# hjmkt/wrenc

Hardware: AMD Instinct MI355X
Metric: all-intra encode fps at fixed QP (CTU RD search + final pass); bit-exactness vs the CPU oracle is checked in `parity` (higher is better)
Workload: dtype u8/i16/i32 (+i64 trellis costs, f32 RD cost)

## Files before the change

### wrenc_amd/csrc/dev_common.h

```cpp
#pragma once
#include <cstddef>
#include <type_traits>

#include "dev_const.h"

namespace wrenc {

enum { PLANAR = 0, DC = 1, LT_CCLM = 81, L_CCLM = 82, T_CCLM = 83 };
enum { TREE_SINGLE = 0, TREE_DUAL_LUMA = 1, TREE_DUAL_CHROMA = 2 };

#define GLOBAL_AS __attribute__((address_space(1)))
#define CONST_AS __attribute__((address_space(4)))
#define AS_GLOBAL(T, p) ((GLOBAL_AS T*)(p))
#define LDS_AS __attribute__((address_space(3)))

constexpr int kReconSlots = 4;
constexpr int kSlotBytes = 1536;
__host__ __device__ constexpr int slot_offset(int slot) { return slot < 2 ? slot * kSlotBytes : (slot == 2 ? 2 * kSlotBytes : 2 * kSlotBytes + 384); }
constexpr int kWaveScratch = 2 * kSlotBytes + 384 + 128;

constexpr int kOrgTile = 1536;
constexpr int kBorderBytes = 272;
struct PicBufs {
    const uint8_t* org[3];
// ... 220 lines not shown
        uint32_t lev_was[4];
    };
    union {
        float split_cost[4];
        uint32_t lev_now[4];
    };
    uint8_t ns_luma[4], ns_chroma[4], child[4];
    CtuSt st;
    XRes xr[2];
};

struct Ctx {
    const CONST_AS DevConst* k;
    const GLOBAL_AS uint8_t* org;
    int W, WH;
    uint8_t* pred_scratch;
    GLOBAL_AS uint8_t* slots;
    unsigned long long* mismatch;
    int ctu_x, ctu_y;
    int cu32_mode;
    int write;
    int member;
    int store;
    int solo;
    int trace;
};

#ifndef WRENC_WPB
#define WRENC_WPB 4
#endif
constexpr int WPB = WRENC_WPB;
constexpr int kWorkgroupsPerCU = 20 / WPB;
constexpr int kTeam = 4;
struct LvBox {
    float ns_cost[3], split[3];
    uint8_t ml[3], mc[3];
    uint16_t pad_;
    uint32_t cnt[3][2];
    uint32_t srv_ready, job_posted, job_done, job_ack, job_fin;
    uint32_t job4_posted, job4_done, job4_ack, job4_fin;
    uint8_t job_bx, job_by, job4_bx, job4_by;
};
struct LdsTab {
    int32_t ldq[256];
    int32_t lv[256];
    int8_t fc[32][4];
    LvBox lvb;
#ifdef WRENC_EXP_LDS_PAD
    char pad[WRENC_EXP_LDS_PAD];
#endif
};
__shared__ Lds SHW[WPB];
__shared__ LdsTab SHT;
#define WAVE (__builtin_amdgcn_readfirstlane((int)(threadIdx.x >> 6)))
#define SH (SHW[WAVE])

__device__ __forceinline__ Ctx uni(Ctx c) {
    c.ctu_x = uni(c.ctu_x);
    c.ctu_y = uni(c.ctu_y);
    c.cu32_mode = uni(c.cu32_mode);
    c.write = uni(c.write);
    c.member = uni(c.member);
    c.store = uni(c.store);
    c.solo = uni(c.solo);
    c.trace = uni(c.trace);
    return c;
}

#define WRENC_PRAGMA_(x) _Pragma(#x)
#define WRENC_UNROLL(n) WRENC_PRAGMA_(unroll n)
#ifndef WRENC_U_DCT
#define WRENC_U_DCT 1
#endif
#ifndef WRENC_U_SAD
#define WRENC_U_SAD 0
#endif

#define WSYNC()                                                  \
    do {                                                         \
        __builtin_amdgcn_fence(__ATOMIC_ACQ_REL, "wavefront");   \
        __builtin_amdgcn_wave_barrier();                         \
    } while (0)

#ifdef WRENC_PROFILE
enum { PH_PREDICT, PH_FDCT, PH_QPRE, PH_QBACK, PH_QTRACE, PH_DEQ, PH_IDCT, PH_RECON, PH_TOTAL, PH_CTRL, PH_REFS, PH_SKIP, PH_NSTEP, PH_NFULL, PH_PSZ, PH_PSZ_END = PH_PSZ + 8, PH_PCNT, PH_PCNT_END = PH_PCNT + 8, PH_QB_PRE, PH_QB_WAIT1, PH_QB_WALK, PH_QB_WAIT2, PH_XCHG, PH_COPY, PH_CB, PH_CB_END = PH_CB + 32, PH_CBN, PH_CBN_END = PH_CBN + 32, PH_MEM, PH_MEM_END = PH_MEM + 16, PH_ST, PH_ST_END = PH_ST + 48, PH_STN, PH_STN_END = PH_STN + 12, PH_EV, PH_EV_END = PH_EV + 64, PH_EVN, PH_EVN_END = PH_EVN + 64, PH_QZ, PH_QZ_END = PH_QZ + 4, PH_LEAF, PH_LEAF_END = PH_LEAF + 13, PH_L4, PH_L4_END = PH_L4 + 6, PH_HIST, PH_HIST_END = PH_HIST + 64, PH_CUT, PH_CUT_END = PH_CUT + 8, PH_PRED, PH_PRED_END = PH_PRED + 8, PH_REC, PH_REC_END = PH_REC + 4, PH_SPARSE, PH_SPARSE_END = PH_SPARSE + 16, PH_COUNT };
__device__ unsigned long long g_prof[PH_COUNT];
__shared__ unsigned long long s_prof[PH_COUNT];
#define PROF_T0() const unsigned long long prof_t0_ = __builtin_readcyclecounter()
#define PROF_ADD(ph) do { if (threadIdx.x == 0) s_prof[ph] += __builtin_readcyclecounter() - prof_t0_; } while (0)
#define PROF_MARK(var) const unsigned long long var = __builtin_readcyclecounter()
#define PROF_ADD2(ph, a, b) do { if (threadIdx.x == 0) s_prof[ph] += (b) - (a); } while (0)
#define PROF_CNT(ph, n) do { if (threadIdx.x == 0) s_prof[ph] += (unsigned long long)(n); } while (0)
#define PROF_ADDM(k, a, b) do { if (LANE == 0 && WAVE < 4) s_prof[PH_MEM + 4 * (k) + WAVE] += (b) - (a); } while (0)
#else
#define PROF_ADDM(k, a, b)
#define PROF_T0()
#define PROF_ADD(ph)
#define PROF_MARK(var)
#define PROF_ADD2(ph, a, b)
#define PROF_CNT(ph, n)
#endif

#ifdef WRENC_TRACE
constexpr unsigned kTraceMax = 1u << 19;
__device__ unsigned int g_trace_n;
__device__ int g_trace[kTraceMax * 8];
__device__ __forceinline__ void trace_rec(int x, int y, int lg, int tree, int kind, int ml, int mc, int bits) {
    const unsigned idx = atomicAdd(&g_trace_n, 1u);
    if (idx < kTraceMax) {
        int* r = g_trace + (size_t)idx * 8;
        r[0] = x;
        r[1] = y;
        r[2] = lg;
        r[3] = tree;
        r[4] = kind;
        r[5] = ml;
        r[6] = mc;
        r[7] = bits;
    }
}
#define TRACE_REC(...) trace_rec(__VA_ARGS__)
#else
#define TRACE_REC(...) do { } while (0)
#endif

template <int CTRL>
__device__ __forceinline__ int dpp_mov(int v) {
    return __builtin_amdgcn_mov_dpp(v, CTRL, 0xF, 0xF, true);
}
constexpr int kDppSwap1 = 0xB1;
constexpr int kDppSwap2 = 0x4E;
constexpr int kDppRowHalfMirror = 0x141;
constexpr int kDppRowMirror = 0x140;
__device__ __forceinline__ int row_sum_i32(int v) {
    v += dpp_mov<kDppSwap1>(v);
    v += dpp_mov<kDppSwap2>(v);
    v += dpp_mov<kDppRowHalfMirror>(v);
    v += dpp_mov<kDppRowMirror>(v);
// ... 126 lines not shown
```

### wrenc_amd/csrc/dev_search.h

```cpp
#pragma once

namespace wrenc {

enum { K_SADLIST = 0, K_FULL = 1, K_NOP = 2, K_SADSEARCH = 3, K_CCLMSEARCH = 4, K_SERVE8 = 5, K_LEAF8 = 7, K_LEAF16 = 8, K_SPLIT8 = 9, K_SERVE4 = 10,
       K_NODE8 = 11 };
enum { COPY_NONE = 0, COPY_SAVE = 1, COPY_RESTORE = 2, COPY_PULL = 3 };

#if defined(WRENC_TRACE) || defined(WRENC_EXHAUSTIVE_SPLITS)
constexpr bool kSplitCut = false;
#else
constexpr bool kSplitCut = true;
#endif

#if defined(WRENC_TRACE) || defined(WRENC_EXHAUSTIVE_CANDIDATES)
constexpr bool kCandidateCut = false;
#else
constexpr bool kCandidateCut = true;
#endif

struct Req {
    int kind;
    int comps;
    int tx, ty, tlg;
    int ml, mc;
    bool active;
    bool refs0, refs1;
    bool final;
    int stage;
    int copy_from;
    bool xchg;
    int tree;
    int pre_copy, copy_comps, copy_slot, copy_tx, copy_ty, copy_tlg;
    float fcur;
};

struct Res {
    uint32_t ssd_y, ssd_c;
    long long lvl_y, lvl_c;
    float v0;
    float vmin;
    int imin;
    int imin2;
};
__device__ __forceinline__ Res res_none() {
    Res r;
    r.ssd_y = 0;
    r.ssd_c = 0;
    r.lvl_y = 0;
    r.lvl_c = 0;
    r.v0 = r.vmin = 3.40282347e+38f;
    r.imin = 0;
    r.imin2 = 0;
    return r;
}

__device__ __forceinline__ float uni_f(float v) { return __int_as_float(uni(__float_as_int(v))); }

__device__ __forceinline__ unsigned checksum_weight(int i) { return (2u * (unsigned)i + 1u) * 0x9E3779B1u; }
// ... 209 lines not shown
            const unsigned s4 = (unsigned)__builtin_amdgcn_readlane((int)acc, 4), s5 = (unsigned)__builtin_amdgcn_readlane((int)acc, 5);
            const unsigned c0 = e0 != kNoMode ? s0 : kNoSad, c1 = e1 != kNoMode ? s1 : kNoSad;
            const unsigned mn = min(min(cur, c0), c1);
            int d = 0;
            if (cur == mn) {
            } else if (c0 == mn) {
                d = -2;
                cur = c0;
            } else {
                d = 2;
                cur = c1;
            }
            const int elo = d < 0 ? e2 : (d == 0 ? e3 : e4), ehi = d < 0 ? e3 : (d == 0 ? e4 : e5);
            const unsigned slo = d < 0 ? s2 : (d == 0 ? s3 : s4), shi = d < 0 ? s3 : (d == 0 ? s4 : s5);
            const unsigned p0 = elo != kNoMode ? slo : kNoSad, p1 = ehi != kNoMode ? shi : kNoSad;
            cm += d;
            const unsigned mn2 = min(min(cur, p0), p1);
            if (cur == mn2) {
            } else if (p0 == mn2) {
                cm -= 1;
                cur = p0;
            } else {
                cm += 1;
                cur = p1;
            }
            const int ilo = d < 0 ? 2 : (d == 0 ? 3 : 4);
            traced = traced && (LANE < 2 || LANE == ilo || LANE == ilo + 1);
        } else {
            const unsigned c0 = e0 != kNoMode ? s0 : kNoSad, c1 = e1 != kNoMode ? s1 : kNoSad;
            const unsigned mn = min(min(cur, c0), c1);
            if (cur == mn) {
            } else if (c0 == mn) {
                cm -= st;
                cur = c0;
            } else {
                cm += st;
                cur = c1;
            }
        }
        if (c.trace && traced)
            TRACE_REC(c.ctu_x + q.tx, c.ctu_y + q.ty, q.tlg, q.tree, (q.comps & 1) ? 0 : 2, (q.comps & 1) ? my_mode : 0, my_mode,
                      __float_as_int((float)acc));
    }
    cm_out = cm;
    smin_out = cur;
}

__device__ __forceinline__ Res leaf8_search(const Ctx& c, const Req& q, int* overflow);
__device__ __forceinline__ Res leaf16_search(const Ctx& c, const Req& q, int* overflow);
__device__ __forceinline__ Res split8_search(const Ctx& c, const Req& q, int* overflow, int* leaves = nullptr);
__device__ __forceinline__ void fill_maps(int bx, int by, int lg, int luma_mode, int chroma_mode, bool luma, bool chroma);
__device__ __forceinline__ void serve_pack4(const Ctx& c, const Req& q, int* overflow);
__device__ __forceinline__ void serve_pack8(const Ctx& c, const Req& q, int* overflow);

__device__ __forceinline__ int cclm_probe(const Ctx& c, int tx, int ty, int lg, int tree, CclmParams* all) {
    const int lane = lane_fresh();
    const unsigned acc = sad_list_cclm(c, tx, ty, lg, all);
    const unsigned lt = (unsigned)__builtin_amdgcn_readlane((int)acc, 0), t = (unsigned)__builtin_amdgcn_readlane((int)acc, 1),
                   l = (unsigned)__builtin_amdgcn_readlane((int)acc, 2);
    if (c.trace && lane < 3)
        TRACE_REC(c.ctu_x + tx, c.ctu_y + ty, lg, tree, 2, 0, lane == 0 ? LT_CCLM : (lane == 1 ? T_CCLM : L_CCLM),
                  __float_as_int((float)acc));
    return (lt <= t && lt <= l) ? LT_CCLM : (t <= l ? T_CCLM : L_CCLM);
}

__device__ __forceinline__ int cclm_pred4_lane(const Ctx& c, const Req& q, const CclmPick& pick, int pl, int x, int y) {
    int v = 128;
    if (!pick.flat128) {
        const int ds = cclm_ds6(c, q.tx, q.ty, 2 * y, 2 * x, pick.avail_l);
        v = (M24(ds, pl ? pick.a1 : pick.a0) >> (pl ? pick.k1 : pick.k0)) + (pl ? pick.b1 : pick.b0);
        v = min(max(v, 0), 255);
    }
    return v;
}

__device__ __forceinline__ float node8_search(const Ctx& c, int tx, int ty, int* overflow) {
    Req qn = {};
    qn.comps = 3;
    qn.tx = tx;
    qn.ty = ty;
    qn.tlg = 3;
    qn.refs0 = true;
    qn.refs1 = true;
    qn.tree = TREE_SINGLE;
    stage_org_leaf(c, 3, tx, ty, 3);
    const Res ru = leaf8_search(c, qn, overflow);
    const float ns = ru.vmin;
    const int ml = ru.imin, mc = ru.imin2;
    fill_maps(tx, ty, 3, ml, mc, true, true);
    unsigned kept;
    {
        const int lane = lane_fresh();
        kept = (unsigned)rec_get(0, tx + (lane & 7), ty + (lane >> 3));
        if (lane < 32) kept |= (unsigned)rec_get(1 + (lane >> 4), (tx >> 1) + (lane & 3), (ty >> 1) + ((lane & 15) >> 2)) << 8;
    }
    qn.fcur = ns;
    int leaves = 0;
    const float split8 = split8_search(c, qn, overflow, &leaves).vmin;
    if (!(split8 > ns)) return split8;
    if (leaves) {
        const int lane = lane_fresh();
        rec_put(0, tx + (lane & 7), ty + (lane >> 3), (int)(kept & 255u));
        if (lane < 32) rec_put(1 + (lane >> 4), (tx >> 1) + (lane & 3), (ty >> 1) + ((lane & 15) >> 2), (int)(kept >> 8));
        fill_maps(tx, ty, 3, ml, mc, true, true);
    }
    return ns;
}

template <bool TEAM, bool D3>
__device__ __forceinline__ Res evaluate(const Ctx& c, const PicBufs& pb, const Req& q, int* overflow) {
    Res r = res_none();
    PROF_MARK(tcp0_);
    if (q.pre_copy != COPY_NONE)
        copy_block(c, q.pre_copy, q.copy_comps, q.copy_slot, q.copy_tx, q.copy_ty, q.copy_tlg, q.copy_from);
    PROF_MARK(tcp1_);
    PROF_ADD2(PH_COPY, tcp0_, tcp1_);
    if (q.kind == K_NOP) return r;
    if (q.stage) stage_org_leaf(c, q.stage, q.tx, q.ty, q.tlg);
    constexpr bool kNodes = !TEAM && D3;
    if (kNodes && q.kind == K_NODE8) {
        r.vmin = node8_search(c, q.tx, q.ty, overflow);
        return r;
    }
    if (!kNodes && q.kind == K_LEAF8) return leaf8_search(c, q, overflow);
    if (q.kind == K_LEAF16) return leaf16_search(c, q, overflow);
    if (TEAM && D3 && q.kind == K_SPLIT8) return split8_search(c, q, overflow);
    if (TEAM && q.kind == K_SERVE8) {
        serve_pack8(c, q, overflow);
        return r;
    }
    if (TEAM && D3 && q.kind == K_SERVE4) {
        serve_pack4(c, q, overflow);
        return r;
    }
    int mc = q.mc;
    CclmPick cpick_ = CclmPick{};
    if (q.kind == K_CCLMSEARCH) {
        if (q.tlg > 4) stage_org(c, 2, q.tx, q.ty, q.tlg);
        CclmParams call_;
        mc = cclm_probe(c, q.tx, q.ty, q.tlg, q.tree, &call_);
        r.imin = mc;
        cpick_ = cclm_pick(call_, 2 * cclm_mode_index(mc));
    }
    if (q.kind == K_FULL || q.kind == K_CCLMSEARCH) {
#pragma unroll 1
        for (int round = 0; round < 2; ++round) {
            const int cset = q.comps & (1 << round);
            if (!cset) continue;
            if (q.active) {
#pragma unroll 1
                for (int comp = 0; comp < 2; ++comp)
                    if ((cset >> comp) & 1) {
                        PROF_MARK(tf0_);
                        full_front(c, q, comp, comp ? mc : q.ml, 0, cpick_);
                        PROF_MARK(tf1_);
                        PROF_ADD2(PH_PSZ + ((q.tlg - 2) * 2 + comp), tf0_, tf1_);
                        PROF_ADD2(PH_PCNT + ((q.tlg - 2) * 2 + comp), 0, 1);
                    }
            }
            PROF_MARK(ts0_);
            bool any_y = false, any_c = false;
            {
                bool any = false;
                long long lvl = 0;
                if (q.active)
                    lvl = quantize_solo(c, q.tlg - round, round ? 2 : 1, overflow, &any);
                if (round) {
                    r.lvl_c = lvl;
                    any_c = any;
                } else {
                    r.lvl_y = lvl;
                    any_y = any;
                }
            }
            PROF_MARK(ts1_);
            PROF_ADD2(PH_QZ + ((q.tlg - 2) & 3), ts0_, ts1_);
            if (!q.active) {
                PROF_ADD2(PH_SKIP, ts0_, ts1_);
                continue;
            }
#pragma unroll 1
            for (int comp = 0; comp < 2; ++comp) {
                if (!((cset >> comp) & 1)) continue;
                PROF_MARK(tb0_);
                const uint32_t ssd = full_back(c, pb, q, comp, 0, comp ? any_c : any_y);
                PROF_MARK(tb1_);
                PROF_ADD2(PH_PSZ + ((q.tlg - 2) * 2 + comp), tb0_, tb1_);
                if (comp)
                    r.ssd_c = ssd;
                else
                    r.ssd_y = ssd;
            }
        }
        return r;
    }
    PROF_MARK(tr0_);
    if (q.refs0 && (q.comps & 1)) build_refs(c, 0, q.tx, q.ty, q.tlg);
    if (q.refs1 && (q.comps & 2)) build_refs(c, 1, q.tx, q.ty, q.tlg);
    if (q.tlg > 4) stage_org(c, q.comps, q.tx, q.ty, q.tlg);
    PROF_MARK(t0_);
    PROF_ADD2(PH_REFS, tr0_, t0_);
    if (q.kind == K_SADSEARCH) {
        constexpr unsigned kNoSad = 0xFFFFFFFFu;
        int cm;
        unsigned smin = kNoSad;
        sad_search(c, q, cm, smin);
        r.imin = uni(cm);
        r.vmin = smin == kNoSad ? 3.40282347e+38f : uni_f((float)smin);
    } else {
        PROF_MARK(tp0_);
        const unsigned sad = (unsigned)wave_sum_i32(predict_sad(c, 1, q.tx, q.ty, q.tlg, q.mc));
        PROF_MARK(tp1_);
        PROF_ADD2(PH_PSZ + ((q.tlg - 2) * 2 + 1), tp0_, tp1_);
        PROF_ADD2(PH_PCNT + ((q.tlg - 2) * 2 + 1), 0, 1);
        if (c.trace && LANE == 0)
            TRACE_REC(c.ctu_x + q.tx, c.ctu_y + q.ty, q.tlg, q.tree, 2, 0, q.mc, __float_as_int((float)sad));
        r.v0 = uni_f((float)sad);
    }
    PROF_MARK(t1_);
    PROF_ADD2(PH_PREDICT, t0_, t1_);
    PROF_ADD2(PH_PRED + 7, t0_, t1_);
    return r;
}

__device__ __forceinline__ int nb_luma_mode(Ctx c, int x, int y, bool* exists) {
    if (x >= 0 && y >= 0) {
        *exists = true;
        return c.cu32_mode;
    }
    if (y >= 0 && x < 0 && c.ctu_x > 0) {
        *exists = true;
        return uni((int)SH.left_mode[y >> 2]);
    }
    *exists = false;
    return PLANAR;
}

struct MpmList {
    int k0, k1, k2, k3, k4;
};
__device__ __forceinline__ MpmList mpm_list(const Ctx& c, int bx, int by, int lg) {
    const int n = 1 << lg;
    bool le, ae;
    int left = nb_luma_mode(c, bx - 1, by + n - 1, &le);
    if (!le) left = PLANAR;
    int above;
    if (by - 1 < 0) {
        above = PLANAR;
// ... 727 lines not shown
}

__device__ __forceinline__ Res leaf16_search(const Ctx& c, const Req& q, int* overflow) {
    Res r = res_none();
    const int lane = lane_fresh();
    if (q.refs0) build_refs(c, 0, q.tx, q.ty, 4);
    if (q.refs1) build_refs(c, 1, q.tx, q.ty, 4);
    LeafBest best = leaf_best_init(PLANAR);
    const MpmList mpl_ = mpm_list(c, q.tx, q.ty, 4);
    {
        PROF_MARK(la0_);
        const Pack16Out a = pack16_eval(c, q, 2, PLANAR, DC, overflow);
        leaf_candidate(c, q.tx, q.ty, 4, TREE_SINGLE, mpl_, best, 0, PLANAR, pack_parts(a, 0));
        leaf_candidate(c, q.tx, q.ty, 4, TREE_SINGLE, mpl_, best, 1, DC, pack_parts(a, 1));
        pack16_to_tile(c, q, 2, best.win);
        PROF_MARK(la1_);
        PROF_ADD2(PH_LEAF + 4, la0_, la1_);
    }
    int cm;
    unsigned smin;
    PROF_MARK(ls0_);
    sad_search(c, q, cm, smin);
    PROF_MARK(ls1_);
    PROF_ADD2(PH_LEAF + 5, ls0_, ls1_);
    cm = uni(cm);
    const int lo = !(cm < 3) ? cm - 1 : kNoMode, hi = !(cm + 1 > 66) ? cm + 1 : kNoMode;
    {
        const Pack16Out b = pack16_eval(c, q, 2, cm, lo, overflow);
        best.win = -1;
        leaf_candidate(c, q.tx, q.ty, 4, TREE_SINGLE, mpl_, best, 0, cm, pack_parts(b, 0));
        if (lo != kNoMode) leaf_candidate(c, q.tx, q.ty, 4, TREE_SINGLE, mpl_, best, 1, lo, pack_parts(b, 1));
        if (best.win >= 0) pack16_to_tile(c, q, 2, best.win);
    }
    PROF_MARK(lb1_);
    PROF_ADD2(PH_LEAF + 6, ls1_, lb1_);
    if (hi != kNoMode) {
        const Pack16Out b = pack16_eval(c, q, 1, hi, kNoMode, overflow);
        best.win = -1;
        leaf_candidate(c, q.tx, q.ty, 4, TREE_SINGLE, mpl_, best, 0, hi, pack_parts(b, 0));
        if (best.win >= 0) pack16_to_tile(c, q, 1, best.win);
    }
    PROF_MARK(lc1_);
    PROF_ADD2(PH_LEAF + 7, lb1_, lc1_);
    r.vmin = best.cost;
    r.imin = best.mode;
    r.imin2 = best.mode;
    r.ssd_y = best.e.ssd_y;
    r.ssd_c = best.e.ssd_c;
    r.lvl_y = best.e.lvl_y;
    r.lvl_c = best.e.lvl_c;
    return r;
}

__device__ __forceinline__ void fill_maps(int bx, int by, int lg, int luma_mode, int chroma_mode, bool luma,
                                          bool chroma) {
    const int l4 = lg - 2;
    if (luma && LANE < (1 << (2 * l4))) {
        const int idx = ((by >> 2) + (LANE >> l4)) * 8 + (bx >> 2) + (LANE & ((1 << l4) - 1));
        SH.cu_log2[idx] = (uint8_t)lg;
        SH.luma_mode[idx] = (uint8_t)luma_mode;
    }
    if (chroma) {
        const int l8 = max(l4 - 1, 0);
        if (LANE < (1 << (2 * l8)))
            SH.chroma_mode[((by >> 3) + (LANE >> l8)) * 4 + (bx >> 3) + (LANE & ((1 << l8) - 1))] = (uint8_t)chroma_mode;
    }
    WSYNC();
}


__device__ __forceinline__ bool split_floor_cut(const Ctx& c, float partial, int n, int fi, bool chroma, float unsplit,
                                                float* bound) {
    if (!kSplitCut) return false;
    float b = partial;
    const float f = c.k->split_floor[fi];
    for (int i = 0; i < n; ++i) b = b + f;
    if (chroma) b = b + c.k->split_floor[1];
    b = uni_f(b);
    if (!(b > unsplit)) return false;
    *bound = b;
    return true;
}

__device__ __forceinline__ Res split8_search(const Ctx& c, const Req& q, int* overflow, int* leaves) {
    Res r = res_none();
    float split8 = 0.0f;
#pragma unroll 1
    for (int i8 = 0; i8 < 4; ++i8) {
        Req ql = {};
        ql.comps = 1;
        ql.tx = q.tx + (i8 & 1) * 4;
        ql.ty = q.ty + (i8 >> 1) * 4;
        ql.tlg = 2;
        ql.refs0 = true;
        ql.refs1 = false;
        ql.tree = TREE_DUAL_LUMA;
        if (split_floor_cut(c, split8, 4 - i8, 0, true, q.fcur, &r.vmin)) {
            PROF_ADD2(PH_CUT + 0, 0, 4 - i8);
            PROF_ADD2(PH_CUT + 1, 0, 1);
            PROF_ADD2(PH_CUT + 4, 0, split8 > q.fcur ? 0 : 1);
            return r;
        }
        if (leaves) *leaves = 1;
        PROF_MARK(l4g0_);
        stage_org_leaf(c, 1, ql.tx, ql.ty, 2);
        PROF_MARK(l4g1_);
// ... 6 lines not shown
        PROF_ADD2(PH_CUT + 1, 0, 1);
        PROF_ADD2(PH_CUT + 4, 0, split8 > q.fcur ? 0 : 1);
        return r;
    }
    Req qc = {};
    qc.tx = q.tx;
    qc.ty = q.ty;
    qc.comps = 2;
    qc.tlg = 3;
    qc.ml = 0;
    qc.mc = uni((int)SH.luma_mode[((q.ty + 4) >> 2) * 8 + ((q.tx + 4) >> 2)]);
    qc.refs0 = false;
    qc.refs1 = true;
    qc.tree = TREE_DUAL_CHROMA;
    PROF_MARK(l4c0_);
    stage_org_leaf(c, 2, q.tx, q.ty, 3);
    const Res rc = leafc4_search(c, qc, overflow);
    fill_maps(q.tx, q.ty, 3, 0, rc.imin, false, true);
    PROF_MARK(l4c1_);
    PROF_ADD2(PH_L4 + 4, l4c0_, l4c1_);
    r.vmin = uni_f(split8 + rc.vmin);
    return r;
}

__device__ __forceinline__ void req_full(Req& q, int comps, int tx, int ty, int tlg, int ml, int mc, bool active,
                                         bool refs0, bool refs1, bool final) {
    q.kind = K_FULL;
    q.comps = comps;
    q.tx = tx;
    q.ty = ty;
    q.tlg = tlg;
    q.ml = ml;
    q.mc = mc;
    q.active = active;
    q.refs0 = refs0;
    q.refs1 = refs1;
    q.final = final;
    q.stage = (final && tlg <= 4) ? comps : 0;
    q.pre_copy = COPY_NONE;
    q.xchg = false;
}

__device__ __forceinline__ void req_copy(Req& q, int mode, int comps, int slot, int tx, int ty, int tlg) {
    q.pre_copy = mode;
    q.copy_comps = comps;
    q.copy_slot = slot;
    q.copy_tx = tx;
    q.copy_ty = ty;
    q.copy_tlg = tlg;
    q.copy_from = -1;
}

enum {
    C_START = 0, C_PLANAR = 1, C_DCM = 2, C_LIST = 3, C_F0 = 6, C_F1 = 7, C_F2 = 8, C_CCLM = 11, C_DM = 12,
    C_L8 = 20, C_L16 = 21, C_WINNER = 22
};

__device__ __forceinline__ void leaf_init(LeafSt& s, int bx, int by, int lg, int slot = 0) {
    s.cont = C_START;
    s.bx = (uint8_t)bx;
    s.by = (uint8_t)by;
    s.lg = (uint8_t)lg;
    s.need_refs0 = 1;
    s.need_refs1 = 1;
    s.need_org = lg <= 4 ? 1 : 0;
    s.need_save = 0;
    s.tile_best = 0;
    s.slot = (uint8_t)slot;
}

__device__ __forceinline__ void leaf_attach_save(LeafSF& s, Req& q) {
    q.pre_copy = COPY_NONE;
    if (s.need_save) {
        req_copy(q, COPY_SAVE, 3, s.slot, s.bx, s.by, s.lg);
        s.need_save = 0;
    }
}
__device__ __forceinline__ void leaf_attach_org(LeafSF& s, Req& q) {
    q.stage = 0;
    if (s.need_org) {
        q.stage = 3;
        s.need_org = 0;
    }
}
__device__ __forceinline__ void leaf_copy_only(LeafSF& s, Req& q, int mode, int comps, int cont) {
    q.kind = K_NOP;
    q.xchg = false;
    req_copy(q, mode, comps, s.slot, s.bx, s.by, s.lg);
    s.cont = (uint8_t)cont;
}

__device__ __forceinline__ void leaf_full(LeafSF& s, Req& q, int comps, int ml, int mc, bool act, int cont) {
    const bool r0 = (comps & 1) && s.need_refs0 != 0;
    const bool r1 = (comps & 2) && mc < LT_CCLM && s.need_refs1 != 0;
    req_full(q, comps, s.bx, s.by, s.lg, ml, mc, act, r0, r1, false);
    q.tree = TREE_SINGLE;
    leaf_attach_org(s, q);
    leaf_attach_save(s, q);
    if (act) {
        if (r0) s.need_refs0 = 0;
        if (r1) s.need_refs1 = 0;
    }
    s.op_ml = (uint8_t)ml;
    s.op_mc = (uint8_t)mc;
    s.op_act = act ? 1 : 0;
    s.cont = (uint8_t)cont;
}
// ... 23 lines not shown
    q.kind = K_SADSEARCH;
    q.xchg = false;
    q.tree = TREE_SINGLE;
    q.comps = 3;
    q.tx = s.bx;
    q.ty = s.by;
    q.tlg = s.lg;
    q.refs0 = s.need_refs0 != 0;
    q.refs1 = s.need_refs1 != 0;
    if (q.refs0) s.need_refs0 = 0;
    if (q.refs1) s.need_refs1 = 0;
    leaf_attach_org(s, q);
    leaf_attach_save(s, q);
    s.cont = (uint8_t)cont;
}

__device__ __forceinline__ void leaf_leaf8(LeafSF& s, Req& q, int cont) {
    req_full(q, 3, s.bx, s.by, s.lg, 0, 0, true, s.need_refs0 != 0, s.need_refs1 != 0, false);
    q.kind = K_LEAF8;
    q.tree = TREE_SINGLE;
    leaf_attach_org(s, q);
    leaf_attach_save(s, q);
    s.need_refs0 = 0;
    s.need_refs1 = 0;
    s.cont = (uint8_t)cont;
}

__device__ __forceinline__ void leaf_leaf16(LeafSF& s, Req& q, int cont) {
    leaf_leaf8(s, q, cont);
    q.kind = K_LEAF16;
}

__device__ __forceinline__ EvalParts res_parts(const Res& r) {
    EvalParts e;
    e.ssd_y = r.ssd_y;
    e.ssd_c = r.ssd_c;
    e.lvl_y = r.lvl_y;
    e.lvl_c = r.lvl_c;
    return e;
}
__device__ __forceinline__ void put_parts(EvalPartsSF& d, const EvalParts& e) {
    d.ssd_y = e.ssd_y;
    d.ssd_c = e.ssd_c;
    d.lvl_y = e.lvl_y;
    d.lvl_c = e.lvl_c;
}

__device__ __forceinline__ void leaf_take(LeafSF& s, float val, const EvalParts& parts, int mode, int cls) {
    s.best_cost = val;
    put_parts(s.e_best, parts);
    s.mode = (uint8_t)mode;
    s.best_cls = (uint8_t)cls;
}
__device__ __forceinline__ void leaf_offer(LeafSF& s, float val, const EvalParts& parts, int mode, int cls) {
    if (val < s.best_cost) {
        leaf_take(s, val, parts, mode, cls);
        s.need_save = 1;
        s.tile_best = 1;
    } else if (s.op_act) {
        s.tile_best = 0;
    }
}

__device__ __forceinline__ bool leaf_step(const Ctx& c, LeafSF& s, const Res& r, Req& q) {
    constexpr int tree = TREE_SINGLE;
    int cont = s.cont;
    float val = 0.0f;
    int cls = 0;
    const EvalParts rp = res_parts(r);
    if (cont == C_PLANAR || cont == C_DCM || cont == C_F0 || cont == C_F1 || cont == C_F2) {
        if (s.op_act) {
            cls = mpm_class(c, s.bx, s.by, s.lg, s.op_ml);
            val = uni_f(assemble_cost(c, tree, cls, s.op_mc, rp));
            if (c.trace && LANE == 0)
                TRACE_REC(c.ctu_x + s.bx, c.ctu_y + s.by, s.lg, tree, 1, s.op_ml, s.op_mc, __float_as_int(val));
        } else {
            val = 3.40282347e+38f;
        }
    }
    for (;;) {
        switch (cont) {
        case C_START:
            if (s.lg == 3) {
                leaf_leaf8(s, q, C_L8);
                return true;
            }
            if (s.lg == 4) {
                leaf_leaf16(s, q, C_L16);
                return true;
            }
            leaf_full(s, q, 3, PLANAR, PLANAR, true, C_PLANAR);
            return true;
        case C_L16:
            leaf_take(s, r.vmin, rp, r.imin, mpm_class(c, s.bx, s.by, s.lg, r.imin));
            s.need_save = 1;
            s.tile_best = 1;
            cont = C_WINNER;
            break;
        case C_L8:
            s.cost = r.vmin;
            s.luma_mode = (uint8_t)r.imin;
            s.chroma_mode = (uint8_t)r.imin2;
            return false;
        case C_PLANAR:
            leaf_take(s, val, rp, PLANAR, cls);
            s.need_save = 1;
            s.tile_best = 1;
            leaf_full(s, q, 3, DC, DC, true, C_DCM);
            return true;
        case C_DCM:
            leaf_offer(s, val, rp, DC, cls);
            leaf_sadsearch(s, q, C_LIST);
            return true;
        case C_LIST: {
            const int cm = r.imin;
            s.cur_mode = (uint8_t)cm;
            s.cur_cost = r.vmin;
            leaf_full(s, q, 3, cm, cm, true, C_F0);
            return true;
        }
        case C_F0: {
            const int cm = s.cur_mode;
            leaf_offer(s, val, rp, cm, cls);
            leaf_full(s, q, 3, cm - 1, cm - 1, !(cm < 3), C_F1);
            return true;
        }
        case C_F1: {
            const int cm = s.cur_mode;
            leaf_offer(s, val, rp, cm - 1, cls);
            leaf_full(s, q, 3, cm + 1, cm + 1, !(cm + 1 > 66), C_F2);
            return true;
        }
        case C_F2:
            leaf_offer(s, val, rp, s.cur_mode + 1, cls);
            cont = C_WINNER;
            break;
        case C_WINNER: {
            s.cost = s.best_cost;
            const int m = s.mode;
            s.luma_mode = (uint8_t)m;
            s.chroma_mode = (uint8_t)m;
            const bool in_tile = s.tile_best != 0;
            s.cur_cost = uni_f(assemble_chroma_cost(c, m, s.e_best.get()));
            if (c.trace && LANE == 0)
                TRACE_REC(c.ctu_x + s.bx, c.ctu_y + s.by, s.lg, tree, 3, 0, m, __float_as_int((float)s.cur_cost));
            leaf_cclmsearch(s, q, C_CCLM);
            if (!in_tile) req_copy(q, COPY_RESTORE, 1, s.slot, s.bx, s.by, s.lg);
            return true;
        }
        case C_CCLM: {
            s.cclm_mode = (uint8_t)r.imin;
            EvalParts e = s.e_best.get();
            e.ssd_c = rp.ssd_c;
            e.lvl_c = rp.lvl_c;
            const float cclm_cost = uni_f(assemble_chroma_cost(c, s.cclm_mode, e));
            if (c.trace && LANE == 0)
                TRACE_REC(c.ctu_x + s.bx, c.ctu_y + s.by, s.lg, tree, 3, 0, s.cclm_mode, __float_as_int(cclm_cost));
            const int m = s.mode;
            const int bcls = s.best_cls;
            if (dm_keeps(s.cur_cost, cclm_cost)) {
                s.cost = uni_f(assemble_cost(c, tree, bcls, m, s.e_best.get()));
                leaf_copy_only(s, q, COPY_RESTORE, 2, C_DM);
                return true;
            }
            s.chroma_mode = s.cclm_mode;
            s.cost = uni_f(assemble_cost(c, tree, bcls, s.cclm_mode, e));
            return false;
        }
        default:
            return false;
        }
    }
}



__device__ __forceinline__ EvalParts xparts(const Ctx& c, int par, int m) {
    const XRes& x = team_lds(c, m).xr[par];
    EvalParts e;
    e.ssd_y = (uint32_t)uni((int)x.ssd_y);
    e.ssd_c = (uint32_t)uni((int)x.ssd_c);
    e.lvl_y = uni_i64(x.lvl_y);
    e.lvl_c = uni_i64(x.lvl_c);
    return e;
}
__device__ __forceinline__ float xvmin(const Ctx& c, int par, int m) { return __int_as_float(uni((int)team_lds(c, m).xr[par].ssd_y)); }
__device__ __forceinline__ int ximin(const Ctx& c, int par, int m) { return uni((int)team_lds(c, m).xr[par].ssd_c); }
__device__ __forceinline__ float xv0(const Ctx& c, int par, int m) { return __int_as_float(uni((int)team_lds(c, m).xr[par].lvl_y)); }

// ... 213 lines not shown
    const int lg = tlg - 1;
    const int cwords = 1 << (2 * lg - 2);
    for (int w = LANE; w < 2 * cwords; w += 64) {
        const int pl = w >= cwords ? 1 : 0;
        const int ww = w - pl * cwords;
        const int row = (4 * ww) >> lg, col = (4 * ww) & ((1 << lg) - 1);
        const int at = ((ty >> 1) + row) * 20 + (tx >> 1) + col + 4;
        *(uint32_t*)&SH.recC[pl][at] = *(const uint32_t*)&src.recC[pl][at];
    }
    WSYNC();
}
__device__ __forceinline__ float lv_decide(const Ctx& c, int L, int idx) {
    const int me = c.member;
    const int dl = c.k->max_depth;
    const int nmem = L == 0 ? kTeam : dl - L + 1;
    PROF_MARK(tx0_);
    lv_meet(L, 0, (idx + 1) * nmem);
    PROF_MARK(tx1_);
    PROF_ADD2(PH_XCHG, tx0_, tx1_);
    PROF_ADDM(2, tx0_, tx1_);
    const float ns = uni_f(SHT.lvb.ns_cost[L]), sp = uni_f(SHT.lvb.split[L]);
    const int ml = uni((int)SHT.lvb.ml[L]), mc = uni((int)SHT.lvb.mc[L]);
    int bx, by;
    lv_node(L, idx, bx, by);
    const int lg = 5 - L;
    const bool unsplit = sp > ns;
    if (unsplit) {
        if (me > L) lv_pull(c, L, bx, by, lg);
        fill_maps(bx, by, lg, ml, mc, true, true);
    } else if (me == L || me > dl) {
        lv_pull(c, L + 1, bx, by, lg);
        lv_pull_maps(c, L + 1, bx, by, lg);
    }
    PROF_MARK(tx2_);
    lv_meet(L, 1, (idx + 1) * nmem);
    PROF_MARK(tx3_);
    PROF_ADD2(PH_COPY, tx1_, tx2_);
    PROF_ADD2(PH_XCHG, tx2_, tx3_);
    PROF_ADDM(2, tx2_, tx3_);
    return unsplit ? ns : sp;
}
__device__ __forceinline__ void lv_post_unsplit(int L, float ns, int ml, int mc) {
    if (LANE == 0) {
        SHT.lvb.ns_cost[L] = ns;
        SHT.lvb.ml[L] = (uint8_t)ml;
        SHT.lvb.mc[L] = (uint8_t)mc;
    }
}
__device__ __forceinline__ void lv_post_split(int L, float sp) {
    if (LANE == 0) SHT.lvb.split[L] = sp;
}


enum { T_START = 0, T_ENTER = 1, T_NODE_LEAF = 2, T_NODE8 = 3, T_REGEN_DONE = 6, T_RETURN = 7, T_FINAL_Z = 8, T_FZ_TAIL = 9, T_FZ_NEXT = 10,
       T_LV_UNIT = 11, T_LV_LEAFDONE = 12, T_LV_UP = 13, T_SPLIT8 = 14, T_LV_SERVE = 15 };

template <bool TEAM, bool D3>
__device__ __forceinline__ bool ctu_step(Ctx& c, const Res& r, Req& q) {
    CtuSt& t = SH.st;
    bool in_leaf = t.in_leaf != 0;
    int cont = t.cont;
    for (;;) {
        if (in_leaf) {
            LeafSF ls = snap_leaf(t.leaf);
            if ((TEAM && !t.lvmode) ? leaf_step_team(c, t, ls, q, t.xpar ^ 1, r) : leaf_step(c, ls, r, q)) {
                if (t.pend) {
                    req_copy(q, COPY_SAVE, t.pend, t.pslot, t.pbx, t.pby, t.plg);
                    t.pend = 0;
                }
                t.cont = (uint8_t)cont;
                t.in_leaf = 1;
                return true;
            }
            t.in_leaf = 0;
            in_leaf = false;
        }
        switch (cont) {
        case T_START:
            t.level = 0;
            t.bx = 0;
            t.by = 0;
            cont = T_ENTER;
            break;
        case T_ENTER: {
            const int lg = 5 - t.level;
            t.lg = (uint8_t)lg;
            if (!TEAM && D3 && lg == 3) {
                req_full(q, 3, t.bx, t.by, 3, 0, 0, true, false, false, false);
                q.kind = K_NODE8;
                q.tree = TREE_SINGLE;
                if (t.pend) {
                    req_copy(q, COPY_SAVE, t.pend, t.pslot, t.pbx, t.pby, t.plg);
                    t.pend = 0;
                }
                t.cont = T_NODE8;
                return true;
            }
            leaf_init(t.leaf, t.bx, t.by, lg, (!TEAM && t.level < t.max_depth) ? 1 + t.level : 0);
            if (TEAM && !t.lvmode) t.leaf.cont = TC_START;
            in_leaf = true;
            cont = T_NODE_LEAF;
            break;
        }
        case T_NODE_LEAF: {
            const float ns = t.leaf.cost;
            const int ml = t.leaf.luma_mode, mc = t.leaf.chroma_mode;
            const int level = t.level, lg = t.lg;
            fill_maps(t.bx, t.by, lg, ml, mc, true, true);
            if (level == 0) c.cu32_mode = ml;
            if (t.max_depth - level == 0) {
                t.ret = ns;
                cont = T_RETURN;
                break;
            }
            if (TEAM) {
                if (t.dp0) {
                    const int dp = t.dp0, dq = t.dp1;
                    t.dp0 = 0;
                    copy_block(c, COPY_PULL, (dp >> 1) & 3, 0, (dq & 7) << 2, (dq >> 3) << 2, (dp >> 5) + 2, (dp >> 3) & 3);
                }
                t.lvmode = 1;
                t.lv_i = 0;
                t.lv_acc0 = 0.0f;
                t.lv_acc1 = 0.0f;
                if (c.member == 0) lv_post_unsplit(0, ns, ml, mc);
                cont = (c.member == 0 || c.member > t.max_depth) ? T_LV_UP : T_LV_UNIT;
                break;
            }
            t.pend = (uint8_t)(mc >= LT_CCLM ? 2 : 0);
            t.pbx = t.bx;
            t.pby = t.by;
            t.plg = (uint8_t)lg;
            t.pslot = (uint8_t)(1 + level);
            if (LANE == 0) {
                SH.ns_cost[level] = ns;
                SH.ns_luma[level] = (uint8_t)ml;
                SH.ns_chroma[level] = (uint8_t)mc;
                SH.split_cost[level] = 0.0f;
                SH.child[level] = 0;
            }
            WSYNC();
            float bound;
            if (split_floor_cut(c, 0.0f, 4, 2 + level + 1, false, ns, &bound)) {
                PROF_ADD2(PH_CUT + 2 + level, 0, 4);
                PROF_ADD2(PH_CUT + 5, 0, 1);
                t.pend = 0;
                t.ret = ns;
                cont = T_RETURN;
                break;
            }
            t.level = (uint8_t)(level + 1);
            cont = T_ENTER;
            break;
        }
        case T_NODE8: {
            if constexpr (!TEAM && D3) {
                t.ret = r.vmin;
                cont = T_RETURN;
                break;
            }
            }
            break;
        case T_SPLIT8: {
            if constexpr (TEAM && D3) {
                lv_post_split(2, r.vmin);
                cont = T_LV_UP;
                break;
            }
            }
            break;
        case T_REGEN_DONE:
            fill_maps(t.rbx, t.rby, t.rlg, t.rl, t.rc, true, true);
            t.ret = uni_f(SH.ns_cost[t.level]);
            cont = T_RETURN;
            break;
        case T_RETURN: {
            const int level = t.level;
            if (level == 0) {
                t.ctu_cost = t.ret;
                t.z = 0;
                if (TEAM && t.dp0) {
                    q.kind = K_NOP;
                    q.pre_copy = COPY_NONE;
                    q.xchg = false;
                    t.cont = T_RETURN;
                    return true;
                }
                t.z = (uint8_t)(TEAM ? 16 * c.member : 0);
                t.zend = (uint8_t)(TEAM ? 16 * c.member + 16 : 64);
                cont = T_FINAL_Z;
                break;
            }
            const int pl = level - 1;
            const int psz = 1 << (5 - pl);
            const int pbx = t.bx & ~(psz - 1), pby = t.by & ~(psz - 1);
            const float acc = uni_f(uni_f(SH.split_cost[pl]) + t.ret);
            const int ch = uni((int)SH.child[pl]) + 1;
            WSYNC();
            if (LANE == 0) {
                SH.split_cost[pl] = acc;
                SH.child[pl] = (uint8_t)ch;
            }
            WSYNC();
            const float ns_p = uni_f(SH.ns_cost[pl]);
            float bound;
            const bool lost = ch < 4 ? split_floor_cut(c, acc, 4 - ch, 2 + level, false, ns_p, &bound) : acc > ns_p;
            if (ch < 4 && !lost) {
// ... 385 lines not shown
```

Baseline: 277.0.

## Run the 32x32 leaf search as one fused device request instead of state-machine steps

Adds a K_LEAF32 request kind that evaluates the whole 32x32 leaf (planar, DC, SAD search, the cm±1 neighbours, then DM vs CCLM chroma) inside a single full_search call. Previously each candidate was a separate request that returned through the ctu_step/leaf_step state machine. The aim is to cut per-request dispatch, state save/restore and snapshot overhead at the CTU level. It removes the old C_PLANAR..C_F2 leaf states and adds profiling slots plus an LDS size static_assert, at the cost of more code and register pressure in the solo path.

```diff
diff --git a/wrenc_amd/csrc/dev_common.h b/wrenc_amd/csrc/dev_common.h
--- a/wrenc_amd/csrc/dev_common.h
+++ b/wrenc_amd/csrc/dev_common.h
@@ -296,6 +296,9 @@
 };
 __shared__ Lds SHW[WPB];
 __shared__ LdsTab SHT;
+#if !defined(WRENC_EXP_LDS_PAD) && WRENC_WPB == 4
+static_assert(sizeof(Lds) * WPB + sizeof(LdsTab) == 31968, "the workgroup's LDS is 31,968 bytes");
+#endif
 #define WAVE (__builtin_amdgcn_readfirstlane((int)(threadIdx.x >> 6)))
 #define SH (SHW[WAVE])
 
@@ -327,7 +330,7 @@
     } while (0)
 
 #ifdef WRENC_PROFILE
-enum { PH_PREDICT, PH_FDCT, PH_QPRE, PH_QBACK, PH_QTRACE, PH_DEQ, PH_IDCT, PH_RECON, PH_TOTAL, PH_CTRL, PH_REFS, PH_SKIP, PH_NSTEP, PH_NFULL, PH_PSZ, PH_PSZ_END = PH_PSZ + 8, PH_PCNT, PH_PCNT_END = PH_PCNT + 8, PH_QB_PRE, PH_QB_WAIT1, PH_QB_WALK, PH_QB_WAIT2, PH_XCHG, PH_COPY, PH_CB, PH_CB_END = PH_CB + 32, PH_CBN, PH_CBN_END = PH_CBN + 32, PH_MEM, PH_MEM_END = PH_MEM + 16, PH_ST, PH_ST_END = PH_ST + 48, PH_STN, PH_STN_END = PH_STN + 12, PH_EV, PH_EV_END = PH_EV + 64, PH_EVN, PH_EVN_END = PH_EVN + 64, PH_QZ, PH_QZ_END = PH_QZ + 4, PH_LEAF, PH_LEAF_END = PH_LEAF + 13, PH_L4, PH_L4_END = PH_L4 + 6, PH_HIST, PH_HIST_END = PH_HIST + 64, PH_CUT, PH_CUT_END = PH_CUT + 8, PH_PRED, PH_PRED_END = PH_PRED + 8, PH_REC, PH_REC_END = PH_REC + 4, PH_SPARSE, PH_SPARSE_END = PH_SPARSE + 16, PH_COUNT };
+enum { PH_PREDICT, PH_FDCT, PH_QPRE, PH_QBACK, PH_QTRACE, PH_DEQ, PH_IDCT, PH_RECON, PH_TOTAL, PH_CTRL, PH_REFS, PH_SKIP, PH_NSTEP, PH_NFULL, PH_PSZ, PH_PSZ_END = PH_PSZ + 8, PH_PCNT, PH_PCNT_END = PH_PCNT + 8, PH_QB_PRE, PH_QB_WAIT1, PH_QB_WALK, PH_QB_WAIT2, PH_XCHG, PH_COPY, PH_CB, PH_CB_END = PH_CB + 32, PH_CBN, PH_CBN_END = PH_CBN + 32, PH_MEM, PH_MEM_END = PH_MEM + 16, PH_ST, PH_ST_END = PH_ST + 48, PH_STN, PH_STN_END = PH_STN + 12, PH_EV, PH_EV_END = PH_EV + 64, PH_EVN, PH_EVN_END = PH_EVN + 64, PH_QZ, PH_QZ_END = PH_QZ + 4, PH_LEAF, PH_LEAF_END = PH_LEAF + 16, PH_L4, PH_L4_END = PH_L4 + 6, PH_HIST, PH_HIST_END = PH_HIST + 64, PH_CUT, PH_CUT_END = PH_CUT + 8, PH_PRED, PH_PRED_END = PH_PRED + 8, PH_REC, PH_REC_END = PH_REC + 4, PH_SPARSE, PH_SPARSE_END = PH_SPARSE + 16, PH_COUNT };
 __device__ unsigned long long g_prof[PH_COUNT];
 __shared__ unsigned long long s_prof[PH_COUNT];
 #define PROF_T0() const unsigned long long prof_t0_ = __builtin_readcyclecounter()
diff --git a/wrenc_amd/csrc/dev_search.h b/wrenc_amd/csrc/dev_search.h
--- a/wrenc_amd/csrc/dev_search.h
+++ b/wrenc_amd/csrc/dev_search.h
@@ -3,7 +3,7 @@
 namespace wrenc {
 
 enum { K_SADLIST = 0, K_FULL = 1, K_NOP = 2, K_SADSEARCH = 3, K_CCLMSEARCH = 4, K_SERVE8 = 5, K_LEAF8 = 7, K_LEAF16 = 8, K_SPLIT8 = 9, K_SERVE4 = 10,
-       K_NODE8 = 11 };
+       K_NODE8 = 11, K_LEAF32 = 12 };
 enum { COPY_NONE = 0, COPY_SAVE = 1, COPY_RESTORE = 2, COPY_PULL = 3 };
 
 #if defined(WRENC_TRACE) || defined(WRENC_EXHAUSTIVE_SPLITS)
@@ -319,6 +319,8 @@
 __device__ __forceinline__ void fill_maps(int bx, int by, int lg, int luma_mode, int chroma_mode, bool luma, bool chroma);
 __device__ __forceinline__ void serve_pack4(const Ctx& c, const Req& q, int* overflow);
 __device__ __forceinline__ void serve_pack8(const Ctx& c, const Req& q, int* overflow);
+template <bool TEAM, bool L32>
+__device__ __forceinline__ Res full_search(const Ctx& c, const PicBufs& pb, const Req& q, int* overflow);
 
 __device__ __forceinline__ int cclm_probe(const Ctx& c, int tx, int ty, int lg, int tree, CclmParams* all) {
     const int lane = lane_fresh();
@@ -400,67 +402,9 @@
         serve_pack4(c, q, overflow);
         return r;
     }
-    int mc = q.mc;
-    CclmPick cpick_ = CclmPick{};
-    if (q.kind == K_CCLMSEARCH) {
-        if (q.tlg > 4) stage_org(c, 2, q.tx, q.ty, q.tlg);
-        CclmParams call_;
-        mc = cclm_probe(c, q.tx, q.ty, q.tlg, q.tree, &call_);
-        r.imin = mc;
-        cpick_ = cclm_pick(call_, 2 * cclm_mode_index(mc));
-    }
-    if (q.kind == K_FULL || q.kind == K_CCLMSEARCH) {
-#pragma unroll 1
-        for (int round = 0; round < 2; ++round) {
-            const int cset = q.comps & (1 << round);
-            if (!cset) continue;
-            if (q.active) {
-#pragma unroll 1
-                for (int comp = 0; comp < 2; ++comp)
-                    if ((cset >> comp) & 1) {
-                        PROF_MARK(tf0_);
-                        full_front(c, q, comp, comp ? mc : q.ml, 0, cpick_);
-                        PROF_MARK(tf1_);
-                        PROF_ADD2(PH_PSZ + ((q.tlg - 2) * 2 + comp), tf0_, tf1_);
-                        PROF_ADD2(PH_PCNT + ((q.tlg - 2) * 2 + comp), 0, 1);
-                    }
-            }
-            PROF_MARK(ts0_);
-            bool any_y = false, any_c = false;
-            {
-                bool any = false;
-                long long lvl = 0;
-                if (q.active)
-                    lvl = quantize_solo(c, q.tlg - round, round ? 2 : 1, overflow, &any);
-                if (round) {
-                    r.lvl_c = lvl;
-                    any_c = any;
-                } else {
-                    r.lvl_y = lvl;
-                    any_y = any;
-                }
-            }
-            PROF_MARK(ts1_);
-            PROF_ADD2(PH_QZ + ((q.tlg - 2) & 3), ts0_, ts1_);
-            if (!q.active) {
-                PROF_ADD2(PH_SKIP, ts0_, ts1_);
-                continue;
-            }
-#pragma unroll 1
-            for (int comp = 0; comp < 2; ++comp) {
-                if (!((cset >> comp) & 1)) continue;
-                PROF_MARK(tb0_);
-                const uint32_t ssd = full_back(c, pb, q, comp, 0, comp ? any_c : any_y);
-                PROF_MARK(tb1_);
-                PROF_ADD2(PH_PSZ + ((q.tlg - 2) * 2 + comp), tb0_, tb1_);
-                if (comp)
-                    r.ssd_c = ssd;
-                else
-                    r.ssd_y = ssd;
-            }
-        }
-        return r;
-    }
+    if (!TEAM && q.kind == K_LEAF32) return full_search<TEAM, true>(c, pb, q, overflow);
+    if (q.kind == K_FULL || q.kind == K_CCLMSEARCH) return full_search<TEAM, false>(c, pb, q, overflow);
+    if constexpr (!TEAM) return r;
     PROF_MARK(tr0_);
     if (q.refs0 && (q.comps & 1)) build_refs(c, 0, q.tx, q.ty, q.tlg);
     if (q.refs1 && (q.comps & 2)) build_refs(c, 1, q.tx, q.ty, q.tlg);
@@ -1294,6 +1238,151 @@
     return r;
 }
 
+template <bool TEAM, bool L32>
+__device__ __forceinline__ Res full_search(const Ctx& c, const PicBufs& pb, const Req& q, int* overflow) {
+    Res r = res_none();
+    constexpr bool l32 = !TEAM && L32;
+    const int tx = l32 ? 0 : q.tx, ty = l32 ? 0 : q.ty, tlg = l32 ? 5 : q.tlg;
+    Req qe = {};
+    qe.tx = tx;
+    qe.ty = ty;
+    qe.tlg = tlg;
+    qe.tree = q.tree;
+    qe.final = q.final;
+    qe.comps = q.comps;
+    qe.ml = q.ml;
+    qe.active = q.active;
+    qe.refs0 = q.refs0;
+    qe.refs1 = q.refs1;
+    int mc = q.mc;
+    CclmPick cpick_ = CclmPick{};
+    LeafBest best = leaf_best_init(PLANAR);
+    MpmList mpl_ = {};
+    int cm = 0;
+    bool tile_best = false;
+    float dm_cost = 0.0f;
+    if (l32) mpl_ = mpm_list(c, tx, ty, tlg);
+    constexpr int steps = l32 ? 6 : 1;
+#pragma unroll 1
+    for (int k = 0; k < steps; ++k) {
+        PROF_MARK(lk0_);
+        bool probe = !l32 && q.kind == K_CCLMSEARCH;
+        if (l32 && (k == 3 ? cm < 3 : (k == 4 && cm + 1 > 66))) continue;
+        if (l32) {
+            if (k == 2) {
+                PROF_MARK(ls0_);
+                stage_org(c, 3, tx, ty, tlg);
+                unsigned smin;
+                sad_search(c, qe, cm, smin);
+                cm = uni(cm);
+                PROF_MARK(ls1_);
+                PROF_ADD2(PH_LEAF + 14, ls0_, ls1_);
+            }
+            const int mode = k == 0 ? PLANAR : (k == 1 ? DC : (k == 2 ? cm : (k == 3 ? cm - 1 : cm + 1)));
+            qe.ml = mode;
+            mc = mode;
+            qe.refs0 = qe.refs1 = k == 0;
+            if (k == 5) {
+                if (!tile_best) copy_block(c, COPY_RESTORE, 1, q.copy_slot, tx, ty, tlg);
+                dm_cost = uni_f(assemble_chroma_cost(c, best.mode, best.e));
+                if (c.trace && LANE == 0)
+                    TRACE_REC(c.ctu_x + tx, c.ctu_y + ty, tlg, TREE_SINGLE, 3, 0, best.mode, __float_as_int(dm_cost));
+                qe.comps = 2;
+                qe.ml = 0;
+                probe = true;
+            }
+        }
+        PROF_MARK(lkc_);
+        if (probe) {
+            if (tlg > 4) stage_org(c, 2, tx, ty, tlg);
+            CclmParams call_;
+            mc = cclm_probe(c, tx, ty, tlg, q.tree, &call_);
+            r.imin = mc;
+            cpick_ = cclm_pick(call_, 2 * cclm_mode_index(mc));
+        }
+#pragma unroll 1
+        for (int round = 0; round < 2; ++round) {
+            const int cset = qe.comps & (1 << round);
+            if (!cset) continue;
+            if (qe.active) {
+#pragma unroll 1
+                for (int comp = 0; comp < 2; ++comp)
+                    if ((cset >> comp) & 1) {
+                        PROF_MARK(tf0_);
+                        full_front(c, qe, comp, comp ? mc : qe.ml, 0, cpick_);
+                        PROF_MARK(tf1_);
+                        PROF_ADD2(PH_PSZ + ((tlg - 2) * 2 + comp), tf0_, tf1_);
+                        PROF_ADD2(PH_PCNT + ((tlg - 2) * 2 + comp), 0, 1);
+                    }
+            }
+            PROF_MARK(ts0_);
+            bool any_y = false, any_c = false;
+            {
+                bool any = false;
+                long long lvl = 0;
+                if (qe.active)
+                    lvl = quantize_solo(c, tlg - round, round ? 2 : 1, overflow, &any);
+                if (round) {
+                    r.lvl_c = lvl;
+                    any_c = any;
+                } else {
+                    r.lvl_y = lvl;
+                    any_y = any;
+                }
+            }
+            PROF_MARK(ts1_);
+            PROF_ADD2(PH_QZ + ((tlg - 2) & 3), ts0_, ts1_);
+            if (!qe.active) {
+                PROF_ADD2(PH_SKIP, ts0_, ts1_);
+                continue;
+            }
+#pragma unroll 1
+            for (int comp = 0; comp < 2; ++comp) {
+                if (!((cset >> comp) & 1)) continue;
+                PROF_MARK(tb0_);
+                const uint32_t ssd = full_back(c, pb, qe, comp, 0, comp ? any_c : any_y);
+                PROF_MARK(tb1_);
+                PROF_ADD2(PH_PSZ + ((tlg - 2) * 2 + comp), tb0_, tb1_);
+                if (comp)
+                    r.ssd_c = ssd;
+                else
+                    r.ssd_y = ssd;
+            }
+        }
+        if (!l32) continue;
+        EvalParts e;
+        e.ssd_y = r.ssd_y;
+        e.ssd_c = r.ssd_c;
+        e.lvl_y = r.lvl_y;
+        e.lvl_c = r.lvl_c;
+        if (k < 5) {
+            tile_best = leaf_candidate(c, tx, ty, tlg, TREE_SINGLE, mpl_, best, k, qe.ml, e);
+            if (tile_best) copy_block(c, COPY_SAVE, 3, q.copy_slot, tx, ty, tlg);
+            PROF_MARK(lk1_);
+            PROF_ADD2(PH_LEAF + 13, lkc_, lk1_);
+            continue;
+        }
+        const int cclm = mc;
+        e.ssd_y = best.e.ssd_y;
+        e.lvl_y = best.e.lvl_y;
+        const float cclm_cost = uni_f(assemble_chroma_cost(c, cclm, e));
+        if (c.trace && LANE == 0)
+            TRACE_REC(c.ctu_x + tx, c.ctu_y + ty, tlg, TREE_SINGLE, 3, 0, cclm, __float_as_int(cclm_cost));
+        r.imin = best.mode;
+        if (dm_keeps(dm_cost, cclm_cost)) {
+            r.vmin = uni_f(assemble_cost(c, TREE_SINGLE, best.cls, best.mode, best.e));
+            r.imin2 = best.mode;
+            copy_block(c, COPY_RESTORE, 2, q.copy_slot, tx, ty, tlg);
+        } else {
+            r.vmin = uni_f(assemble_cost(c, TREE_SINGLE, best.cls, cclm, e));
+            r.imin2 = cclm;
+        }
+        PROF_MARK(lk2_);
+        PROF_ADD2(PH_LEAF + 15, lk0_, lk2_);
+    }
+    return r;
+}
+
 __device__ __forceinline__ void fill_maps(int bx, int by, int lg, int luma_mode, int chroma_mode, bool luma,
                                           bool chroma) {
     const int l4 = lg - 2;
@@ -1406,7 +1495,7 @@
 }
 
 enum {
-    C_START = 0, C_PLANAR = 1, C_DCM = 2, C_LIST = 3, C_F0 = 6, C_F1 = 7, C_F2 = 8, C_CCLM = 11, C_DM = 12,
+    C_START = 0, C_CCLM = 11, C_DM = 12,
     C_L8 = 20, C_L16 = 21, C_WINNER = 22
 };
 
@@ -1536,32 +1625,10 @@
     s.mode = (uint8_t)mode;
     s.best_cls = (uint8_t)cls;
 }
-__device__ __forceinline__ void leaf_offer(LeafSF& s, float val, const EvalParts& parts, int mode, int cls) {
-    if (val < s.best_cost) {
-        leaf_take(s, val, parts, mode, cls);
-        s.need_save = 1;
-        s.tile_best = 1;
-    } else if (s.op_act) {
-        s.tile_best = 0;
-    }
-}
-
 __device__ __forceinline__ bool leaf_step(const Ctx& c, LeafSF& s, const Res& r, Req& q) {
     constexpr int tree = TREE_SINGLE;
     int cont = s.cont;
-    float val = 0.0f;
-    int cls = 0;
     const EvalParts rp = res_parts(r);
-    if (cont == C_PLANAR || cont == C_DCM || cont == C_F0 || cont == C_F1 || cont == C_F2) {
-        if (s.op_act) {
-            cls = mpm_class(c, s.bx, s.by, s.lg, s.op_ml);
-            val = uni_f(assemble_cost(c, tree, cls, s.op_mc, rp));
-            if (c.trace && LANE == 0)
-                TRACE_REC(c.ctu_x + s.bx, c.ctu_y + s.by, s.lg, tree, 1, s.op_ml, s.op_mc, __float_as_int(val));
-        } else {
-            val = 3.40282347e+38f;
-        }
-    }
     for (;;) {
         switch (cont) {
         case C_START:
@@ -1569,11 +1636,7 @@
                 leaf_leaf8(s, q, C_L8);
                 return true;
             }
-            if (s.lg == 4) {
-                leaf_leaf16(s, q, C_L16);
-                return true;
-            }
-            leaf_full(s, q, 3, PLANAR, PLANAR, true, C_PLANAR);
+            leaf_leaf16(s, q, C_L16);
             return true;
         case C_L16:
             leaf_take(s, r.vmin, rp, r.imin, mpm_class(c, s.bx, s.by, s.lg, r.imin));
@@ -1586,39 +1649,6 @@
             s.luma_mode = (uint8_t)r.imin;
             s.chroma_mode = (uint8_t)r.imin2;
             return false;
-        case C_PLANAR:
-            leaf_take(s, val, rp, PLANAR, cls);
-            s.need_save = 1;
-            s.tile_best = 1;
-            leaf_full(s, q, 3, DC, DC, true, C_DCM);
-            return true;
-        case C_DCM:
-            leaf_offer(s, val, rp, DC, cls);
-            leaf_sadsearch(s, q, C_LIST);
-            return true;
-        case C_LIST: {
-            const int cm = r.imin;
-            s.cur_mode = (uint8_t)cm;
-            s.cur_cost = r.vmin;
-            leaf_full(s, q, 3, cm, cm, true, C_F0);
-            return true;
-        }
-        case C_F0: {
-            const int cm = s.cur_mode;
-            leaf_offer(s, val, rp, cm, cls);
-            leaf_full(s, q, 3, cm - 1, cm - 1, !(cm < 3), C_F1);
-            return true;
-        }
-        case C_F1: {
-            const int cm = s.cur_mode;
-            leaf_offer(s, val, rp, cm - 1, cls);
-            leaf_full(s, q, 3, cm + 1, cm + 1, !(cm + 1 > 66), C_F2);
-            return true;
-        }
-        case C_F2:
-            leaf_offer(s, val, rp, s.cur_mode + 1, cls);
-            cont = C_WINNER;
-            break;
         case C_WINNER: {
             s.cost = s.best_cost;
             const int m = s.mode;
@@ -1938,7 +1968,7 @@
 }
 
 
-enum { T_START = 0, T_ENTER = 1, T_NODE_LEAF = 2, T_NODE8 = 3, T_REGEN_DONE = 6, T_RETURN = 7, T_FINAL_Z = 8, T_FZ_TAIL = 9, T_FZ_NEXT = 10,
+enum { T_START = 0, T_ENTER = 1, T_NODE_LEAF = 2, T_NODE8 = 3, T_LEAF32 = 4, T_REGEN_DONE = 6, T_RETURN = 7, T_FINAL_Z = 8, T_FZ_TAIL = 9, T_FZ_NEXT = 10,
        T_LV_UNIT = 11, T_LV_LEAFDONE = 12, T_LV_UP = 13, T_SPLIT8 = 14, T_LV_SERVE = 15 };
 
 template <bool TEAM, bool D3>
@@ -1982,6 +2012,14 @@
                 t.cont = T_NODE8;
                 return true;
             }
+            if (!TEAM && lg == 5) {
+                req_full(q, 3, t.bx, t.by, 5, 0, 0, true, true, true, false);
+                q.kind = K_LEAF32;
+                q.tree = TREE_SINGLE;
+                q.copy_slot = t.level < t.max_depth ? 1 + t.level : 0;
+                t.cont = T_LEAF32;
+                return true;
+            }
             leaf_init(t.leaf, t.bx, t.by, lg, (!TEAM && t.level < t.max_depth) ? 1 + t.level : 0);
             if (TEAM && !t.lvmode) t.leaf.cont = TC_START;
             in_leaf = true;
@@ -2039,6 +2077,16 @@
             cont = T_ENTER;
             break;
         }
+        case T_LEAF32: {
+            if constexpr (!TEAM) {
+                t.leaf.cost = r.vmin;
+                t.leaf.luma_mode = (uint8_t)r.imin;
+                t.leaf.chroma_mode = (uint8_t)r.imin2;
+                cont = T_NODE_LEAF;
+                break;
+            }
+            }
+            break;
         case T_NODE8: {
             if constexpr (!TEAM && D3) {
                 t.ret = r.vmin;
```

Measured after the change: 281.5 (median of 6 runs). 1.6% higher.
